# sanhue903/CUDA_Selection_Criteria

Measured on AMD Instinct MI355X. Metric: sketch pair-comparisons/sec (N genomes x m buckets), higher is better.
Workload: dtype u64; 1 GPU; cfg3: 10000 genomes, smh_a m=512, tau=0.8; mode smh_a; bands 64 x 8 rows; pair space sharded by query rows over 1 GPU(s), selected pairs all_gathered; n_genomes=10000, m=512, algo=sig, criterion=smh_a, selected_pairs=45000, stage1_survivors=45000, n_ranks_seen=1, stage2_grouping=label order

## Files before the change

cuda_selection_criteria_amd/csrc/abi_context.inc:

```

extern "C" {

const char* selhip_version(void) { return "selhip 0.1 (gfx950)"; }

int selhip_device_count(void) {
    int cnt = 0;
    if (hipGetDeviceCount(&cnt) != hipSuccess) return 0;
    return cnt;
}

const char* selhip_last_error(const selhip_ctx* ctx) {
    if (ctx) return ctx->err.c_str();
    return g_last_error.c_str();
}

int selhip_ctx_create(selhip_ctx** out, int device) {
    if (!out) return SELHIP_E_BADARG;
    *out = nullptr;
    int rc = check_device(nullptr);
    if (rc) return rc;
    int cnt = 0;
    (void)hipGetDeviceCount(&cnt);
    if (device < 0 || device >= cnt) { set_err(nullptr, "device %d out of range (0..%d)", device, cnt - 1); return SELHIP_E_BADARG; }
    HIPCHK(nullptr, hipSetDevice(device));
// ... 2 lines not shown
    if (std::strncmp(prop.gcnArchName, "gfx950", 6) != 0) {
        set_err(nullptr, "device %d is %s; this library is built for gfx950 only", device, prop.gcnArchName);
        return SELHIP_E_NODEVICE;
    }
    selhip_ctx* c = new selhip_ctx();
    c->device = device;
    c->dev_cus = prop.multiProcessorCount;
    *out = c;
    return SELHIP_OK;
}

void selhip_ctx_destroy(selhip_ctx* c) {
    if (!c) return;
    (void)hipSetDevice(c->device);
    (void)hipStreamSynchronize(c->stream);
    drain_timers(c);
    c->own_hll.release(); c->own_aux.release(); c->own_cards.release();
    c->ecard.release(); c->hi.release(); c->pc.buf.release(); c->seg_cnt.release(); c->surv.release();
    c->counts.release(); c->results.release(); c->self_pairs.release();
    c->aux_il.release(); c->cand.release(); c->sig.release(); c->fin.release(); c->own_aux_hll.release();
    c->hj_keys_in.release(); c->hj_keys_out.release(); c->hj_vals_in.release(); c->hj_vals_out.release(); c->hj_tmp.release();
    c->csr_cnt.release(); c->csr_start.release(); c->grouped.release(); c->scan_tmp.release();
    c->planes.release(); c->small_bar.release(); c->mat_row_pos.release(); c->mat_col_pos.release();
    c->hll_sparse.release(); c->hll_sparse_dev_t.release();
    release_queries(c);
    release_topk(c);
    c->gs.release();
    release_merge(c);
    if (c->h_pc) (void)hipHostFree(c->h_pc);
    if (c->st_stage1) {
        (void)hipStreamDestroy(c->st_stage1);
        (void)hipEventDestroy(c->ev_start); (void)hipEventDestroy(c->ev_end);
    }
    delete c;
}

int selhip_ctx_set_stream(selhip_ctx* c, void* hip_stream) {
    if (!c) return SELHIP_E_BADARG;
    if (c->stream != (hipStream_t)hip_stream && c->pc.buf.p) {
        (void)hipStreamSynchronize(c->stream);
        c->pc.dirty = true;
    }
    c->stream = (hipStream_t)hip_stream;
    return SELHIP_OK;
}

int selhip_ctx_set_fp_mode(selhip_ctx* c, int fp_mode) {
// ... 89 lines not shown
        return SELHIP_OK;
    }
    if (!std::strcmp(name, "query_join_tile")) {
        if (value != 16 && value != 32) { set_err(&c->err, "query_join_tile must be 16 or 32"); return SELHIP_E_BADARG; }
        c->query_join_tile = value;
        return SELHIP_OK;
    }
    if (!std::strcmp(name, "timed_kernel")) {
        if (value < 0 || value > 1) { set_err(&c->err, "timed_kernel must be 0 (stage-1 kernel) or 1 (stage 2a)"); return SELHIP_E_BADARG; }
        c->timed_kernel = value;
        return SELHIP_OK;
    }
    if (!std::strcmp(name, "hist_algo")) {
        if (value < -1 || value > 1) { set_err(&c->err, "hist_algo must be -1 (automatic), 0 (byte rows, LDS histogram) or 1 (bit planes)"); return SELHIP_E_BADARG; }
        c->hist_algo = value;
        if (value == 0) c->planes.khi = 0;
        return SELHIP_OK;
    }
    if (!std::strcmp(name, "hist_sparse")) {
        if (value < -1 || value > 1) { set_err(&c->err, "hist_sparse must be -1 (automatic), 0 (every value from the bit planes) or 1 (values >= the set's threshold from its sparse lists)"); return SELHIP_E_BADARG; }
        c->hist_sparse = value;
        return SELHIP_OK;
    }
    if (!std::strcmp(name, "dense_fused")) { c->dense_fused = value != 0; return SELHIP_OK; }
    if (!std::strcmp(name, "matrix_mirror")) { c->matrix_mirror = value != 0; return SELHIP_OK; }
    if (!std::strcmp(name, "matrix_smh_form")) {
        if (value != 1 && value != 3) { set_err(&c->err, "matrix_smh_form: 1 (every pair once, mirrored) or 3 (the whole square)"); return SELHIP_E_BADARG; }
        c->matrix_smh_form = (int)value; return SELHIP_OK;
    }
    if (!std::strcmp(name, "hist_dense_degree")) {
        if (value < -1 || value > (1 << 20)) { set_err(&c->err, "hist_dense_degree must be in [-1, 2^20] (-1 = never)"); return SELHIP_E_BADARG; }
        c->hist_dense_degree = value;
        return SELHIP_OK;
    }
    if (!std::strcmp(name, "hist_bs_blocks")) {
        if (value < 8 || value > 65536 || value % 8) { set_err(&c->err, "hist_bs_blocks must be a multiple of 8 in [8, 65536]"); return SELHIP_E_BADARG; }
        c->hist_bs_blocks = value;
        return SELHIP_OK;
    }
    if (!std::strcmp(name, "hist_blocks")) {
        if (value < 8 || value > 65536 || value % 8) { set_err(&c->err, "hist_blocks must be a multiple of 8 in [8, 65536]"); return SELHIP_E_BADARG; }
        c->hist_blocks = value;
        return SELHIP_OK;
    }
    if (!std::strcmp(name, "cluster_blocks")) {
        if (value < 0 || value > 65536) { set_err(&c->err, "cluster_blocks must be in [0, 65536] (0 = automatic)"); return SELHIP_E_BADARG; }
        g_cluster_blocks.store(value, std::memory_order_relaxed);
        return SELHIP_OK;
    }
    set_err(&c->err, "unknown parameter '%s'", name);
    return SELHIP_E_BADARG;
}

int selhip_ctx_get_param(const selhip_ctx* c, const char* name, int* value) {
    if (!c || !name || !value) return SELHIP_E_BADARG;
    if (!std::strcmp(name, "hll_khi"))          { *value = c->planes.khi; return SELHIP_OK; }
    if (!std::strcmp(name, "hist_bitplanes"))   { *value = use_bitslices(c) ? 1 : 0; return SELHIP_OK; }
    if (!std::strcmp(name, "hist_sparse_t"))    { *value = sparse_t_used(c); return SELHIP_OK; }
    if (!std::strcmp(name, "label_order"))      { *value = label_order(c) ? 1 : 0; return SELHIP_OK; }
    if (!std::strcmp(name, "join_tile_rows"))   { *value = join_tile_rows(c); return SELHIP_OK; }
    if (!std::strcmp(name, "join_form_used"))   { *value = c->join_form_used; return SELHIP_OK; }
    if (!std::strcmp(name, "chunks"))           { *value = c->n_chunks_last; return SELHIP_OK; }
    if (!std::strcmp(name, "dense_route_used")) { *value = c->dense_route_used; return SELHIP_OK; }
    if (!std::strcmp(name, "smhc_path_used"))   { *value = c->smhc_path_used; return SELHIP_OK; }
    if (!std::strcmp(name, "smhc_rule_used"))   { *value = c->smhc_rule_used; return SELHIP_OK; }
    if (!std::strcmp(name, "matrix_mirror"))    { *value = c->matrix_mirror; return SELHIP_OK; }
    if (!std::strcmp(name, "matrix_smh_form"))  { *value = c->matrix_smh_form; return SELHIP_OK; }
    if (!std::strcmp(name, "matrix_smh_path_used")) { *value = c->matrix_smh_path_used; return SELHIP_OK; }
    if (!std::strcmp(name, "clusters_last"))    { *value = c->clusters_last; return SELHIP_OK; }
    if (!std::strcmp(name, "cluster_blocks"))   { *value = g_cluster_blocks.load(std::memory_order_relaxed); return SELHIP_OK; }
    if (!std::strcmp(name, "greedy_clusters_last")) { *value = c->greedy_clusters_last; return SELHIP_OK; }
    if (!std::strcmp(name, "greedy_rounds_last"))   { *value = c->greedy_rounds_last; return SELHIP_OK; }
    if (!std::strcmp(name, "forest_rounds_last"))   { *value = c->forest_rounds_last; return SELHIP_OK; }
    if (!std::strcmp(name, "linkage_rounds_last"))  { *value = c->linkage_rounds_last; return SELHIP_OK; }
    if (!std::strcmp(name, "linkage_merges_last"))  { *value = c->linkage_merges_last; return SELHIP_OK; }
    if (!std::strcmp(name, "linkage_rowscans_last")) { *value = c->linkage_rowscans_last; return SELHIP_OK; }
    if (!std::strcmp(name, "linkage_rescans_last")) { *value = c->linkage_rescans_last; return SELHIP_OK; }
    if (!std::strcmp(name, "forest_edges_last"))    { *value = c->forest_edges_last; return SELHIP_OK; }
    if (!std::strcmp(name, "small_pass_used"))  { *value = c->small_used ? 1 : 0; return SELHIP_OK; }
    if (!std::strcmp(name, "pairs_route_used")) { *value = c->pairs_route_used; return SELHIP_OK; }
    if (!std::strcmp(name, "pairs_gpw"))        { *value = c->pairs_gpw_used; return SELHIP_OK; }
// ... 147 lines not shown
    return SELHIP_OK;
}

static int load_cards(selhip_ctx* c, const char* noun, const uint8_t* d_hll, int64_t n, const double* cards_src, bool cards_on_host,
                      DevBuf<double>& own, const double** d_cards, bool host_cards_checked = false) {
    if (!cards_src) {
        HIPCHK(&c->err, own.ensure((size_t)n));
        const int rc = compute_cards(c, d_hll, n, c->p, own.p);
        if (rc) return rc;
        *d_cards = own.p;
    } else if (cards_on_host) {
        if (!host_cards_checked) { const int rc = check_host_cards(c, noun, cards_src, n); if (rc) return rc; }
        HIPCHK(&c->err, own.ensure((size_t)n));
        HIPCHK(&c->err, hipMemcpyAsync(own.p, cards_src, (size_t)n * sizeof(double), hipMemcpyHostToDevice, c->stream));
        *d_cards = own.p;
    } else {
        *d_cards = cards_src;
    }
    HIPCHK(&c->err, hipStreamSynchronize(c->stream));
    return SELHIP_OK;
}

static int after_sketches(selhip_ctx* c, const double* cards_src, bool cards_on_host) {
    c->planes.khi = 0; c->hll_sparse_t = 0;
    if (c->n == 0) return SELHIP_OK;
    if (c->p == 14 && c->hist_algo != 0) {
        int rc = c->planes.build(&c->err, c->stream, c->d_hll, c->n);
        if (rc) return rc;
        HIPCHK(&c->err, c->hll_sparse.ensure((size_t)c->n * kBsSparseCap));
        HIPCHK(&c->err, c->hll_sparse_dev_t.ensure(1));
        rc = build_sparse_lists(&c->err, c->stream, c->planes.bs.p, c->n, c->hll_sparse.p, c->hll_sparse_dev_t.p, &c->hll_sparse_t);
        if (rc) return rc;
    }
    return load_cards(c, "cards", c->d_hll, c->n, cards_src, cards_on_host, c->own_cards, &c->d_cards, true);
}

static void set_database(selhip_ctx* c, int64_t n, int m, int p_hll) {
    c->n = n; c->m = m; c->p = p_hll; c->have_run = false; c->pending = false; c->cand_begin = 0; c->sig_key = 0; c->small_pass_failed = false;
    c->d_aux_hll = nullptr; c->p_aux = 0;
    drop_queries(c);
}

static int no_database(selhip_ctx* c, int rc) {
    c->n = 0; c->d_hll = nullptr; c->d_aux = nullptr; c->d_cards = nullptr; c->owns_sketches = false;
    c->planes.khi = 0; c->hll_sparse_t = 0;
    return rc;
}

static int upload_rows(selhip_ctx* c, const uint8_t* h_hll, const uint64_t* h_aux, const double* h_cards) {
    const size_t hb = (size_t)1 << c->p;
    if (c->n > 0) {
        HIPCHK(&c->err, c->own_hll.ensure((size_t)c->n * hb));
        HIPCHK(&c->err, c->own_aux.ensure((size_t)c->n * c->m));
        HIPCHK(&c->err, hipMemcpyAsync(c->own_hll.p, h_hll, (size_t)c->n * hb, hipMemcpyHostToDevice, c->stream));
        HIPCHK(&c->err, hipMemcpyAsync(c->own_aux.p, h_aux, (size_t)c->n * c->m * 8, hipMemcpyHostToDevice, c->stream));
    }
    c->d_hll = c->own_hll.p; c->d_aux = (const u64*)c->own_aux.p; c->owns_sketches = true;
    return after_sketches(c, h_cards, true);
}

int selhip_ctx_upload(selhip_ctx* c, const uint8_t* h_hll, const uint64_t* h_aux, const double* h_cards,
                      int64_t n, int m, int p_hll) {
    if (!c) return SELHIP_E_BADARG;
    HIPCHK(&c->err, hipSetDevice(c->device));
    int rc = validate_shape(c, n, m, p_hll);
    if (rc) return rc;
    if (n > 0 && (!h_hll || !h_aux)) { set_err(&c->err, "null sketch pointer"); return SELHIP_E_BADARG; }
    if (h_cards) { rc = check_host_cards(c, "cards", h_cards, n); if (rc) return rc; }
// ... 313 lines not shown
```

cuda_selection_criteria_amd/csrc/host_context.hpp:

```cpp
#pragma once

namespace {

thread_local std::string g_last_error = "";

void set_err(std::string* dst, const char* fmt, ...) {
    char buf[512];
    va_list ap;
    va_start(ap, fmt);
    vsnprintf(buf, sizeof buf, fmt, ap);
    va_end(ap);
    if (dst) *dst = buf;
    g_last_error = buf;
}

#define HIPCHK(ctx_err, expr)                                                                  \
    do {                                                                                       \
        hipError_t e__ = (expr);                                                               \
        if (e__ != hipSuccess) {                                                               \
            set_err(ctx_err, "%s failed: %s (%s:%d)", #expr, hipGetErrorString(e__), __FILE__, __LINE__); \
            return SELHIP_E_HIP;                                                               \
        }                                                                                      \
    } while (0)

// ... 153 lines not shown
    SigSet sig;
    DevBuf<u64> hj_keys_in, hj_keys_out;
    DevBuf<int> hj_vals_in, hj_vals_out;
    DevBuf<char> hj_tmp;
    DevBuf<int> csr_cnt, csr_start;
    DevBuf<selhip_int2_t> grouped;
    DevBuf<char> scan_tmp;
    size_t scan_tmp_stride = 0;
    PassCounters* h_pc = nullptr;
    hipStream_t st_stage1 = nullptr;
    hipEvent_t ev_start = nullptr, ev_end = nullptr;
    int n_chunks_last = 1;
    int pipeline = -1;
    int64_t cand_begin = 0;
    int il_block = 128, il_parts = 1, il_part = 0;
    int hist_pad = 0;
    int hist_run = 0, hist_blocks = kHistSpanBlocks;
    BitPlanes planes;
    DevBuf<u64> small_bar;
    DevBuf<uint32_t> hll_sparse;
    DevBuf<int> hll_sparse_dev_t;
    int hll_sparse_t = 0;
    int hist_sparse = -1;
    int hist_algo = -1;
    int hist_dense_degree = 32;
    int hist_bs_blocks = 2048;
    int group_label = -1;
    int verify_fb = 0;
    int join_wpb = 4;
    int join_db = 1;
    int join_tri = 0;
    int join_form = 2;
    int join_form_used = -1;
    int join_t = 0;
    int join_bits = 16;
    int join_q = 1;
    long long enum_pairs = kEnumPairs;
    int sig_tile_g = 16;
    int sig_cache = 0;
    long long sig_key = 0;
    int sig_tile = 1;
    int init_cap = 0;
    int join_qt = 0;
    bool group_stage2 = true;
    int small_pass = -1;
    bool small_used = false, small_pass_failed = false;
// ... 191 lines not shown
```

cuda_selection_criteria_amd/csrc/host_pairs.hpp:

```cpp
#pragma once

namespace {

constexpr long long kPairsSigShare = 2;

int pairs_route(const selhip_ctx* c, bool smh, int algo, int n_rows, int n_bands, int64_t n_pairs) {
    if (!smh) return 2;
    if (algo == SELHIP_ALGO_STREAM || !sig_supported(n_rows, n_bands)) return 0;
    if (algo == SELHIP_ALGO_SIG) return 1;
    const bool cached = c->sig_cache && c->sig_key == sig_cache_key(c, n_rows, n_bands);
    return cached || n_pairs >= c->n / kPairsSigShare ? 1 : 0;
}

hipError_t launch_pairs_filter(selhip_ctx* c, u64 off, u64 end, double tau, selhip_int2_t* out, u64 out_cap, u64* out_count, PassCounters* pc0) {
    const unsigned grid = grid_for(end - off, kPairsBlock, kPairsMaxGrid);
    if (off == 0) c->pairs_grid_used = (int)grid;
    hipLaunchKernelGGL(pairs_filter_kernel, dim3(grid), dim3(kPairsBlock), 0, c->stream,
                       c->list_pairs, off, end, (int)c->n, c->ecard.p, tau, c->mode == SELHIP_MODE_CB_SMH ? 1 : 0, out, out_cap, out_count, pc0);
    return hipGetLastError();
}

int enqueue_pairs_pass(selhip_ctx* c) {
    const int n = (int)c->n;
    const double tau = (double)c->tau_f;
    const int crit = c->criterion;
    const int use_cb = c->mode == SELHIP_MODE_CB_SMH ? 1 : 0;
    const u64 P = (u64)c->list_n;
    c->dominant_timer = c->timed_kernel == 1 ? T_HIST : T_STAGE1;
    if (c->timing) c->timed_passes += 1;
    TimerScope total(c, T_TOTAL);
    CounterSets::Claim pcs;
    HIPCHK(&c->err, c->pc.claim(c->stream, &pcs));
    c->pcb = pcs.cur;
    PassCounters* const pc0 = c->pcb;
    if (c->fail_after_flip) { c->fail_after_flip = 0; set_err(&c->err, "test hook: enqueue failed after the counter flip"); return SELHIP_E_HIP; }
    c->small_used = false;
    c->n_chunks_last = 1;
    if (c->pairs_route_used == 1) {
        HIPCHK(&c->err, launch_sig_build(c, c->n_rows, c->n_bands, tau, 0, 0, pcs.next));
    } else {
        TimerScope t(c, T_PREP);
        hipLaunchKernelGGL(cb_bounds_kernel, dim3((unsigned)((n + 255) / 256)), dim3(256), 0, c->stream,
                           c->d_cards, n, tau, use_cb, row_map(c, 0, 0), c->ecard.p, c->hi.p, pc0,
                           grouping_on(c) && !c->plan.emit ? c->csr_cnt.p : nullptr, grouping_on(c) && !c->plan.emit ? (int)c->csr_cnt.cap : 0, 0, pcs.next,
                           c->seg_cnt.p, (int)c->seg_cnt.cap);
        HIPCHK(&c->err, hipGetLastError());
    }
    const Chain ch = chain_slices(c, 0, 1, c->stream, 0, n, pc0, false);
    const StageIO& io = ch.io;
    const selhip_int2_t* final_list = io.surv;
    const u64* final_count = &io.pc->n_survivors;
    u64 final_cap = io.cap;
    if (c->plan.smh) {
        {
            TimerScope t(c, T_STAGE1);
            const unsigned grid = grid_for(P, kPairsBlock, kPairsMaxGrid);
            c->pairs_gpw_used = 0; c->pairs_grid_used = (int)grid;
            if (c->plan.count) {
                const PairsDirectShape sh = pairs_direct_shape(P);
// ... 61 lines not shown
```

cuda_selection_criteria_amd/csrc/host_pass.hpp:

```cpp
#pragma once

namespace {

template <int NCH, int LOG2R>
hipError_t launch_stream(selhip_ctx* c, const StageIO& io, const RowMap& rm) {
    constexpr int Q = kQueryVgprBudget / NCH;
    const int n = (int)c->n;
    const long long n_tiles_ll = rm.n_tiles(Q);
    if (n_tiles_ll > 0x7FFFFFFFll) return hipErrorInvalidValue;
    const int n_tiles = (int)n_tiles_ll;
    const int chunk_base = ((rm.row_begin + 1) / kChunk) * kChunk;
    const int n_chunks = (n - chunk_base + kChunk - 1) / kChunk;
    if (n_tiles <= 0 || n_chunks <= 0) return hipSuccess;
    const long long blocks = (long long)n_tiles * n_chunks;
    if (blocks > 0x7FFFFFFFll) return hipErrorInvalidValue;
    hipLaunchKernelGGL((smh_stream_kernel<NCH, LOG2R>), dim3((unsigned)blocks), dim3(kBlock), 0, io.st,
                       reinterpret_cast<const u64x2*>(c->aux_il.p), n, c->hi.p, c->pcb,
                       rm, n_tiles, chunk_base, io.surv, io.cap, io.pc);
    return hipGetLastError();
}

template <int NCH, int LOG2R>
hipError_t launch_stream_r(selhip_ctx* c, const StageIO& io, int l, const RowMap& rm) {
    if (l == LOG2R) return launch_stream<NCH, LOG2R>(c, io, rm);
// ... 377 lines not shown
template <int NB>
void launch_hist_bs_nb(int g1, unsigned blocks, hipStream_t st, const uint32_t* bs, const uint8_t* gmax, const uint32_t* lists, const selhip_int2_t* list,
                       const u64* count, u64 cap, uint32_t* counts, u64 off, u64 window, int run, u64 dense_pairs) {
#define SELHIP_BS_LAUNCH(G1) hipLaunchKernelGGL((hll_union_hist_bs_kernel<NB, G1>), dim3(blocks), dim3(kBlock), 0, st, bs, gmax, lists, list, count, cap, \
                                                counts, off, window, run, dense_pairs)
    switch (g1) {
        case 1: SELHIP_BS_LAUNCH(1); return;
        case 2: SELHIP_BS_LAUNCH(2); return;
        case 3: SELHIP_BS_LAUNCH(3); return;
    }
    if constexpr (NB > 4) {
        switch (g1) {
            case 4: SELHIP_BS_LAUNCH(4); return;
            case 5: SELHIP_BS_LAUNCH(5); return;
        }
    }
    if constexpr (NB > 5) {
        if (g1 == 6) { SELHIP_BS_LAUNCH(6); return; }
    }
    SELHIP_BS_LAUNCH(0);
#undef SELHIP_BS_LAUNCH
}
hipError_t launch_hist_bs(int khi, unsigned blocks, hipStream_t st, const uint32_t* bs, const uint8_t* gmax, const selhip_int2_t* list, const u64* count,
                          u64 cap, uint32_t* counts, u64 off, u64 window, int run, u64 dense_pairs, int sparse_t = 0, const uint32_t* lists = nullptr) {
    const int g1 = sparse_t > 0 && sparse_t < khi && lists ? sparse_t / 4 : 0;
    switch (bs_planes(khi)) {
        case 4:  launch_hist_bs_nb<4>(g1, blocks, st, bs, gmax, lists, list, count, cap, counts, off, window, run, dense_pairs); break;
        case 5:  launch_hist_bs_nb<5>(g1, blocks, st, bs, gmax, lists, list, count, cap, counts, off, window, run, dense_pairs); break;
        default: launch_hist_bs_nb<6>(g1, blocks, st, bs, gmax, lists, list, count, cap, counts, off, window, run, dense_pairs);
    }
    return hipGetLastError();
}

int build_sparse_lists(std::string* err, hipStream_t st, const uint32_t* d_bs, int64_t n, uint32_t* d_lists, int* d_t, int* t) {
    *t = 0;
    if (n <= 0) return SELHIP_OK;
    HIPCHK(err, hipMemsetAsync(d_t, 0, sizeof(int), st));
    hipLaunchKernelGGL(hll_sparse_t_kernel, dim3(grid_for((u64)n, kWavesPerBlock, 8192)), dim3(kBlock), 0, st, d_bs, (long long)n, d_t);
    HIPCHK(err, hipGetLastError());
    int need = 0;
    HIPCHK(err, hipMemcpyAsync(&need, d_t, sizeof(int), hipMemcpyDeviceToHost, st));
    HIPCHK(err, hipStreamSynchronize(st));
    if (need < 4 || need > kBsSparseMaxT) return SELHIP_OK;
    hipLaunchKernelGGL(hll_sparse_list_kernel, dim3(grid_for((u64)n, kWavesPerBlock, 8192)), dim3(kBlock), 0, st, d_bs, (long long)n, need, d_lists);
    HIPCHK(err, hipGetLastError());
    HIPCHK(err, hipStreamSynchronize(st));
    *t = need;
    return SELHIP_OK;
}

bool use_bitslices(const selhip_ctx* c) { return c->p == 14 && c->planes.khi > 0 && c->hist_algo != 0; }
constexpr size_t kSparseMaxPlaneBytes = (size_t)192 << 20;
int sparse_t_used(const selhip_ctx* c) {
    if (!use_bitslices(c) || !c->hist_sparse || c->hll_sparse_t >= c->planes.khi) return 0;
    if (c->hist_sparse < 0 && (size_t)c->n * kBsGenomeDwords * sizeof(uint32_t) > kSparseMaxPlaneBytes) return 0;
    if (c->hll_sparse_t > 20 && c->planes.khi <= 32) return 0;
    return c->hll_sparse_t;
}

int compute_cards(selhip_ctx* c, const uint8_t* d_hll, int64_t n, int p, double* d_out) {
    if (n <= 0) return SELHIP_OK;
    HIPCHK(&c->err, c->self_pairs.ensure((size_t)n));
    HIPCHK(&c->err, c->counts.ensure((size_t)n * 64));
    hipLaunchKernelGGL(iota_pairs_kernel, dim3((unsigned)((n + 255) / 256)), dim3(256), 0, c->stream, c->self_pairs.p, (int)n);
    HIPCHK(&c->err, hipGetLastError());
    hipLaunchKernelGGL(hll_union_hist_kernel, dim3(grid_for((u64)n, kWavesPerBlock, 4096)), dim3(kBlock), 0, c->stream,
                       d_hll, p, c->self_pairs.p, (const u64*)nullptr, (u64)n, (u64)n, c->counts.p);
    HIPCHK(&c->err, hipGetLastError());
    HIPCHK(&c->err, launch_select<0>(c->fp_mode == SELHIP_FP_FMA, c->stream, grid_for((u64)n, kWave, 8192), c->counts.p,
                                     nullptr, (u64)n, (u64)n, p, d_out, nullptr, nullptr, 0.0, nullptr, 0, nullptr,
                                     nullptr, nullptr));
    return SELHIP_OK;
}

long long pair_bound(long long n, long long rb, long long re) {
    long long cnt = 0;
    const long long rows = re - rb;
    cnt = rows * (n - 1) - (rb + re - 1) * rows / 2;
    return cnt < 0 ? 0 : cnt;
}

// ... 54 lines not shown
    selhip_int2_t* fin; u64 fin_cap;
    int* csr_cnt; int* csr_start; char* scan_tmp;
    selhip_int2_t* grouped;
    uint32_t* counts; u64 window;
};

size_t csr_stride(int n) { return 5 * (size_t)n + 2; }

constexpr double kLabelOrderPairs = 4e8;
constexpr size_t kLabelOrderBytes = (size_t)192 << 20;
bool label_order(const selhip_ctx* c) {
    if (!grouping_on(c)) return false;
    if (c->group_label >= 0) return c->group_label == 1;
    if (use_bitslices(c)) return true;
    return (size_t)c->n * 16384 > kLabelOrderBytes && (double)pair_bound(c->n, c->row_begin, c->row_end) / std::max(1, c->il_parts) >= kLabelOrderPairs;
}

int enqueue_hist_select(selhip_ctx* c, const Chain& ch, const selhip_int2_t* final_list, const u64* final_count, u64 final_cap,
                        bool grouped, double tau, PassCounters* pc0) {
    hipStream_t st = ch.io.st;
    for (u64 off = 0; off < final_cap; off += ch.window) {
        {
            TimerScope t(c, T_HIST, st);
            if (use_bitslices(c))
                HIPCHK(&c->err, launch_hist_bs(c->planes.khi, (unsigned)c->hist_bs_blocks, st, c->planes.bs.p, c->planes.gmax.p, final_list, final_count, final_cap, ch.counts, off, ch.window,
                                               c->hist_run > 0 ? c->hist_run : (grouped ? 4 : 1),
                                               grouped && c->hist_dense_degree >= 0
                                                   ? (u64)c->hist_dense_degree * (u64)std::max<long long>(1, ((long long)ch.re - ch.rb) / std::max(1, c->il_parts)) : ~0ull,
                                               sparse_t_used(c), c->hll_sparse.p));
            else if (c->p == 14)
                hipLaunchKernelGGL(hll_union_hist_runs_kernel, dim3(c->hist_blocks), dim3(kWave), (size_t)c->hist_pad, st,
                                   c->d_hll, final_list, final_count, final_cap, ch.counts, off, ch.window,
                                   c->hist_run > 0 ? c->hist_run : (grouped && label_order(c) ? 4 : 1));
            else
                hipLaunchKernelGGL(hll_union_hist_kernel, dim3(2048), dim3(kBlock), 0, st,
                                   c->d_hll, c->p, final_list, final_count, (u64)0, final_cap, ch.counts, off, ch.window);
            HIPCHK(&c->err, hipGetLastError());
        }
        TimerScope t(c, T_SELECT, st);
        HIPCHK(&c->err, launch_select<1>(c->fp_mode == SELHIP_FP_FMA, st, 4096, ch.counts, final_count, 0,
                                         final_cap, c->p, nullptr, final_list, c->ecard.p, tau,
                                         c->results.p, (u64)c->results.cap, pc0, nullptr, nullptr, off, ch.window, c->measure));
    }
    return SELHIP_OK;
}

int enqueue_tail(selhip_ctx* c, const Chain& ch, const selhip_int2_t* final_list, const u64* final_count, u64 final_cap,
                 bool counted, double tau, PassCounters* pc0) {
    const int n = (int)c->n;
    hipStream_t st = ch.io.st;
    const bool grouped = grouping_on(c);
    if (grouped) {
// ... 176 lines not shown
    ch.counts = c->counts.p + (size_t)k * ch.window * 64;
    if (count_in_verify) { ch.io.row_cnt = ch.csr_cnt; if (label_order(c)) ch.io.row_lab = ch.csr_cnt + 2 * (size_t)n; }
    return ch;
}

int enqueue_pass(selhip_ctx* c) {
    const int n = (int)c->n;
    const int rb = (int)(c->rd.on ? c->rd.begin : c->row_begin), re = (int)(c->rd.on ? c->rd.end : c->row_end);
    const double tau = (double)c->tau_f;
    const int crit = c->criterion;
    const PassPlan& plan = c->plan;
    c->dominant_timer = c->timed_kernel == 1 ? T_HIST : crit == SELHIP_CRIT_NONE ? T_DENSE : (plan.use_sig ? T_JOIN : T_STAGE1);
    if (c->timing && !(c->rd.on && c->rd.begin != c->row_begin)) c->timed_passes += 1;
    TimerScope total(c, T_TOTAL);
    const bool smh_crit = plan.smh, use_hash = plan.use_hash, use_sig = plan.use_sig;
    if (plan.bad) { set_err(&c->err, plan.bad, c->n_rows, c->n_bands); return SELHIP_E_BADARG; }
    CounterSets::Claim pcs;
    HIPCHK(&c->err, c->pc.claim(c->stream, &pcs));
    c->pcb = pcs.cur;
    PassCounters* const pc_next = pcs.next;
    PassCounters* pc0 = c->pcb;
    if (c->fail_after_flip) { c->fail_after_flip = 0; set_err(&c->err, "test hook: enqueue failed after the counter flip"); return SELHIP_E_HIP; }
    c->small_used = small_pass_ok(c);
    if (c->small_used) {
        c->n_chunks_last = 1;
        const int rc = enqueue_small_pass(c, pc_next, tau);
        if (rc) return rc;
        HIPCHK(&c->err, hipMemcpyAsync(c->h_pc, c->pcb, sizeof(PassCounters) * (kMaxChunks + 1), hipMemcpyDeviceToHost, c->stream));
        c->pc.dirty = false;
        return SELHIP_OK;
    }
    if (use_sig) {
        HIPCHK(&c->err, launch_sig_build(c, c->n_rows, c->n_bands, tau, rb, re, pc_next));
    } else {
        TimerScope t(c, T_PREP);
        hipLaunchKernelGGL(cb_bounds_kernel, dim3((unsigned)((n + 255) / 256)), dim3(256), 0, c->stream,
                           c->d_cards, n, tau, c->mode == SELHIP_MODE_CB_SMH ? 1 : 0, row_map(c, rb, re), c->ecard.p, c->hi.p, pc0,
                           grouping_on(c) && !plan.emit ? c->csr_cnt.p : nullptr, grouping_on(c) && !plan.emit ? (int)c->csr_cnt.cap : 0, (int)c->cand_begin, pc_next,
                           c->seg_cnt.p, (int)c->seg_cnt.cap);
        HIPCHK(&c->err, hipGetLastError());
        if (plan.il_stream) {
            const int nch = c->m / 128;
            const long long total = (long long)c->n * nch * kWave;
            hipLaunchKernelGGL(stream_interleave_kernel, dim3((unsigned)((total + kBlock - 1) / kBlock)), dim3(kBlock), 0, c->stream,
                               reinterpret_cast<const u64x2*>(c->d_aux), reinterpret_cast<u64x2*>(c->aux_il.p), total, nch);
            HIPCHK(&c->err, hipGetLastError());
// ... 146 lines not shown
```

cuda_selection_criteria_amd/csrc/kernel_hllbs.cuh:

```cuda
#pragma once

namespace {

constexpr int kBsPlanes = 6;
constexpr int kBsPlaneDwords = 512;
constexpr int kBsGenomeDwords = kBsPlanes * kBsPlaneDwords;

__global__ __launch_bounds__(kBlock)
void hll_bitslice_kernel(const uint8_t* __restrict__ hll, long long n, uint32_t* __restrict__ bs, uint8_t* __restrict__ gmax,
                         int* __restrict__ max_val) {
    const int lane = threadIdx.x & (kWave - 1);
    uint32_t mx_all = 0;
    for (long long g = (long long)blockIdx.x * kWavesPerBlock + threadIdx.x / kWave; g < n; g += (long long)gridDim.x * kWavesPerBlock) {
        const uint32_t* row = reinterpret_cast<const uint32_t*>(hll + g * 16384);
        uint32_t* dst = bs + g * kBsGenomeDwords;
        uint32_t mx = 0;
#pragma unroll 1
        for (int o = 0; o < 8; ++o) {
            uint32_t d[8];
#pragma unroll
            for (int jj = 0; jj < 8; ++jj) d[jj] = row[(o * 8 + jj) * kWave + lane] & 0x3F3F3F3Fu;
            uint32_t out[kBsPlanes];
#pragma unroll
            for (int b = 0; b < kBsPlanes; ++b) out[b] = 0;
#pragma unroll
            for (int jj = 0; jj < 8; ++jj) {
                const uint32_t w = d[jj];
                mx = max(max(mx, w & 0xFFu), max((w >> 8) & 0xFFu, max((w >> 16) & 0xFFu, w >> 24)));
#pragma unroll
// ... 30 lines not shown
        int cnt[6] = {0, 0, 0, 0, 0, 0};
#pragma unroll 1
        for (int o = 0; o < kBsPlaneDwords / kWave; ++o) {
            uint32_t p[kBsPlanes];
#pragma unroll
            for (int b = 0; b < kBsPlanes; ++b) p[b] = src[b * kBsPlaneDwords + o * kWave + lane];
#pragma unroll
            for (int k = 1; k <= 6; ++k) cnt[k - 1] += __popc(bs_ge4k(p, k));
        }
        int t = kBsSparseMaxT + 4;
#pragma unroll
        for (int k = 6; k >= 1; --k) {
            int s = cnt[k - 1];
#pragma unroll
            for (int d = 32; d > 0; d >>= 1) s += __shfl_xor(s, d, kWave);
            if (s <= kBsSparseCap) t = 4 * k;
        }
        t_all = max(t_all, t);
    }
    if (lane == 0 && t_all) atomicMax(t_need, t_all);
}

__global__ __launch_bounds__(kBlock)
void hll_sparse_list_kernel(const uint32_t* __restrict__ bs, long long n, int t, uint32_t* __restrict__ lists) {
    const int lane = threadIdx.x & (kWave - 1);
    for (long long g = (long long)blockIdx.x * kWavesPerBlock + threadIdx.x / kWave; g < n; g += (long long)gridDim.x * kWavesPerBlock) {
        const uint32_t* src = bs + g * kBsGenomeDwords;
        uint32_t* dst = lists + g * kBsSparseCap;
        int base = 0;
#pragma unroll 1
        for (int o = 0; o < kBsPlaneDwords / kWave; ++o) {
            const int d = o * kWave + lane;
            uint32_t p[kBsPlanes];
#pragma unroll
            for (int b = 0; b < kBsPlanes; ++b) p[b] = src[b * kBsPlaneDwords + d];
            uint32_t h = bs_ge4k(p, t >> 2);
            const int cnt = __popc(h);
            int incl = cnt;
#pragma unroll
            for (int s = 1; s < kWave; s <<= 1) {
                const int v = __shfl_up(incl, s, kWave);
                if (lane >= s) incl += v;
            }
            int off = base + incl - cnt;
            while (h) {
                const int j = __builtin_ctz(h);
                h &= h - 1;
                uint32_t v = 0;
#pragma unroll
                for (int b = 0; b < kBsPlanes; ++b) v |= ((p[b] >> j) & 1u) << b;
                if (off < kBsSparseCap) dst[off] = ((uint32_t)(d * 32 + j) << 8) | v;
                ++off;
            }
            base += __shfl(incl, kWave - 1, kWave);
        }
        for (int i = lane; i < kBsSparseCap; i += kWave)
            if (i >= base) dst[i] = kBsSparseNone;
    }
}

template <int NB>
__device__ __forceinline__ void bs_load(const uint32_t* __restrict__ bs, int g, int lane, uint32_t (&r)[NB][8]) {
    const uint4* p = reinterpret_cast<const uint4*>(bs + (size_t)g * kBsGenomeDwords);
#pragma unroll
    for (int b = 0; b < NB; ++b) {
        const uint4 lo = p[b * (kBsPlaneDwords / 4) + lane], hi = p[b * (kBsPlaneDwords / 4) + kWave + lane];
        r[b][0] = lo.x; r[b][1] = lo.y; r[b][2] = lo.z; r[b][3] = lo.w;
        r[b][4] = hi.x; r[b][5] = hi.y; r[b][6] = hi.z; r[b][7] = hi.w;
    }
}

template <int TBL>
__device__ __forceinline__ uint32_t bs_op3(uint32_t a, uint32_t b, uint32_t c) { return __builtin_amdgcn_bitop3_b32(a, b, c, TBL); }
__device__ __forceinline__ void bs_count(uint32_t& acc, uint32_t mask) {
    asm("v_bcnt_u32_b32 %0, %1, %0" : "+v"(acc) : "v"(mask));
}

template <int NB, int G>
__device__ __forceinline__ uint32_t bs_group_node(const uint32_t (&M)[NB], const uint32_t (&pre)[4]) {
    constexpr int s1 = (G & 2) ? 0xCC : 0x33, s0 = (G & 1) ? 0xAA : 0x55;
    if constexpr (NB == 4)      return bs_op3<((G & 2) ? 0xF0 : 0x0F) & ((G & 1) ? 0xCC : 0x33)>(M[3], M[2], M[2]);
    else if constexpr (NB == 5) return bs_op3<((G & 4) ? 0xF0 : 0x0F) & s1 & s0>(M[4], M[3], M[2]);
    else                        return bs_op3<0xF0 & s1 & s0>(pre[G >> 2], M[3], M[2]);
}

template <int NB, int G0, int G, int GEND>
// ... 150 lines not shown
    }
    const uint32_t hA = sp->bins[my_bin];
    sp->bins[my_bin] = 0u;
    __builtin_amdgcn_fence(__ATOMIC_RELEASE, "wavefront");
    __builtin_amdgcn_wave_barrier();
    __builtin_amdgcn_fence(__ATOMIC_ACQUIRE, "wavefront");
    return hA;
}

__device__ __forceinline__ void bs_sparse_entry(BsSparseLds* sp, uint32_t e) {
    if (e == kBsSparseNone) return;
    const uint32_t r = e >> 8, v = e & 63, w = sp->bits[r >> 5], below = w & ((1u << (r & 31)) - 1u);
    if ((w >> (r & 31)) & 1u) {
        const uint32_t av = sp->val[sp->first[r >> 5] + __popc(below)];
        if (v > av) {
            atomicAdd(&sp->bins[v], 1u);
            atomicSub(&sp->bins[av], 1u);
        }
    } else {
        atomicAdd(&sp->bins[v], 1u);
    }
}

template <int NB, int G1>
__global__ __launch_bounds__(kBlock, NB <= 5 ? 4 : 2)
void hll_union_hist_bs_kernel(const uint32_t* __restrict__ bs, const uint8_t* __restrict__ gmax, const uint32_t* __restrict__ lists,
                              const selhip_int2_t* __restrict__ pairs, const u64* __restrict__ n_pairs_dev, u64 cap, uint32_t* __restrict__ counts,
                              u64 chunk_off, u64 chunk_len, int run_len, u64 dense_pairs) {
    const int lane = threadIdx.x & (kWave - 1);
    const int wave = threadIdx.x / kWave;
    u64 n_pairs = *n_pairs_dev;
    if (n_pairs > cap) n_pairs = cap;
    n_pairs = n_pairs > chunk_off ? min(n_pairs - chunk_off, chunk_len) : 0;
    pairs += chunk_off;
    u64 blocks_active = gridDim.x;
    {
        const u64 resident = 1024ull * (NB <= 5 ? 4 : 2);
        if (n_pairs <= 8 * resident) {
            const u64 waves = min(resident, max(n_pairs, (u64)64));
            blocks_active = min((u64)gridDim.x, ((waves + 8 * kWavesPerBlock - 1) / (8 * kWavesPerBlock)) * 8);
        }
    }
    if (blockIdx.x >= blocks_active) return;
    const u64 stride = (blocks_active >> 3) * kWavesPerBlock;
    const int my_bin = ((lane & 2) ? 32 : 0) + 2 * bs_pidx(lane) + (lane & 1);
    const bool dense = n_pairs >= dense_pairs;
    const uint32_t xcd = blockIdx.x & 7u;
// ... 4 lines not shown
    const u64 n_tasks = (n_pairs + run_len - 1) / run_len;
    const u64 tasks_per_xcd = dense ? n_tasks : (n_tasks + 7) >> 3;
    const u64 t_begin = dense ? 0 : (u64)xcd * tasks_per_xcd, t_end = min(t_begin + tasks_per_xcd, n_tasks);
    int cur_x = -1;
    uint32_t xa[NB][8];
    BsSparseLds* sp = nullptr;
    uint32_t hA = 0;
    if constexpr (G1 > 0) {
        __shared__ BsSparseLds sp_block[kWavesPerBlock];
        sp = &sp_block[wave];
        sp->bins[my_bin] = 0u;
    }
    for (u64 task = t_begin + (u64)(blockIdx.x >> 3) * kWavesPerBlock + wave; task < t_end; task += stride) {
        const u64 j0 = task * run_len;
        const int cnt = (int)min((u64)run_len, n_pairs - j0);
        selhip_int2_t pr{0, 0};
        if (lane < cnt) pr = pairs[j0 + lane];
        u64 mine = __ballot(lane < cnt && (!dense || (((uint32_t)pr.y * 0x9E3779B1u) >> 29) == xcd));
        while (mine) {
            const int src = (int)__builtin_ctzll(mine);
            mine &= mine - 1;
            const int px = __builtin_amdgcn_readlane(pr.x, src), py = __builtin_amdgcn_readlane(pr.y, src);
            uint32_t yb[NB][8];
            bs_load<NB>(bs, py, lane, yb);
            if constexpr (G1 == 0) {
                if (px != cur_x) { bs_load<NB>(bs, px, lane, xa); cur_x = px; }
                const int kp = max((int)gmax[px], (int)gmax[py]) + 1;
                const uint32_t tot = bs_pair_hist<NB>(xa, yb, kp, lane);
                counts[(j0 + src) * 64 + my_bin] = (lane & 1) ? (tot >> 16) : (tot & 0xFFFFu);
            } else {
                const uint32_t eb0 = lists[(size_t)py * kBsSparseCap + lane], eb1 = lists[(size_t)py * kBsSparseCap + kWave + lane];
                if (px != cur_x) { bs_load<NB>(bs, px, lane, xa); hA = bs_sparse_row(sp, lists, px, lane, my_bin); cur_x = px; }
                uint32_t P[16];
#pragma unroll
                for (int v = 0; v < 16; ++v) P[v] = 0u;
                bs_decode<NB, 0, G1, 16>(xa, yb, P);
                const uint32_t tot = bs_reduce16<2 * G1>(P, lane);
                bs_sparse_entry(sp, eb0);
                bs_sparse_entry(sp, eb1);
                __builtin_amdgcn_fence(__ATOMIC_RELEASE, "wavefront");
                __builtin_amdgcn_wave_barrier();
                __builtin_amdgcn_fence(__ATOMIC_ACQUIRE, "wavefront");
                const uint32_t s = sp->bins[my_bin];
                sp->bins[my_bin] = 0u;
                const uint32_t dense_cnt = (lane & 2) ? 0u : ((lane & 1) ? (tot >> 16) : (tot & 0xFFFFu));
                counts[(j0 + src) * 64 + my_bin] = dense_cnt + hA + s;
            }
        }
    }
}


}
```

Measured before the change: 279.4 billion pairs/s.

## Add clamped four-plane HLL image to shrink sparse histogram kernel loads

```diff
diff --git a/cuda_selection_criteria_amd/csrc/abi_context.inc b/cuda_selection_criteria_amd/csrc/abi_context.inc
--- a/cuda_selection_criteria_amd/csrc/abi_context.inc
+++ b/cuda_selection_criteria_amd/csrc/abi_context.inc
@@ -48,7 +48,7 @@
     c->hj_keys_in.release(); c->hj_keys_out.release(); c->hj_vals_in.release(); c->hj_vals_out.release(); c->hj_tmp.release();
     c->csr_cnt.release(); c->csr_start.release(); c->grouped.release(); c->scan_tmp.release();
     c->planes.release(); c->small_bar.release(); c->mat_row_pos.release(); c->mat_col_pos.release();
-    c->hll_sparse.release(); c->hll_sparse_dev_t.release();
+    c->hll_sparse.release(); c->hll_sparse_dev_t.release(); c->hll_image.release();
     release_queries(c);
     release_topk(c);
     c->gs.release();
@@ -184,6 +184,11 @@
         c->hist_sparse = value;
         return SELHIP_OK;
     }
+    if (!std::strcmp(name, "hist_image")) {
+        if (value < -1 || value > 1) { set_err(&c->err, "hist_image must be -1 (automatic), 0 (the six-plane rows) or 1 (the clamped image where the set holds one)"); return SELHIP_E_BADARG; }
+        c->hist_image = value;
+        return SELHIP_OK;
+    }
     if (!std::strcmp(name, "dense_fused")) { c->dense_fused = value != 0; return SELHIP_OK; }
     if (!std::strcmp(name, "matrix_mirror")) { c->matrix_mirror = value != 0; return SELHIP_OK; }
     if (!std::strcmp(name, "matrix_smh_form")) {
@@ -219,6 +224,7 @@
     if (!std::strcmp(name, "hll_khi"))          { *value = c->planes.khi; return SELHIP_OK; }
     if (!std::strcmp(name, "hist_bitplanes"))   { *value = use_bitslices(c) ? 1 : 0; return SELHIP_OK; }
     if (!std::strcmp(name, "hist_sparse_t"))    { *value = sparse_t_used(c); return SELHIP_OK; }
+    if (!std::strcmp(name, "hist_image"))       { *value = c->hist_image_used; return SELHIP_OK; }
     if (!std::strcmp(name, "label_order"))      { *value = label_order(c) ? 1 : 0; return SELHIP_OK; }
     if (!std::strcmp(name, "join_tile_rows"))   { *value = join_tile_rows(c); return SELHIP_OK; }
     if (!std::strcmp(name, "join_form_used"))   { *value = c->join_form_used; return SELHIP_OK; }
@@ -412,14 +418,14 @@
 }
 
 static int after_sketches(selhip_ctx* c, const double* cards_src, bool cards_on_host) {
-    c->planes.khi = 0; c->hll_sparse_t = 0;
+    c->planes.khi = 0; c->hll_sparse_t = 0; c->hll_image_ok = false;
     if (c->n == 0) return SELHIP_OK;
     if (c->p == 14 && c->hist_algo != 0) {
         int rc = c->planes.build(&c->err, c->stream, c->d_hll, c->n);
         if (rc) return rc;
         HIPCHK(&c->err, c->hll_sparse.ensure((size_t)c->n * kBsSparseCap));
         HIPCHK(&c->err, c->hll_sparse_dev_t.ensure(1));
-        rc = build_sparse_lists(&c->err, c->stream, c->planes.bs.p, c->n, c->hll_sparse.p, c->hll_sparse_dev_t.p, &c->hll_sparse_t);
+        rc = build_sparse_lists(&c->err, c->stream, c->planes.bs.p, c->n, c->hll_sparse.p, c->hll_sparse_dev_t.p, &c->hll_sparse_t, &c->hll_image, &c->hll_image_ok);
         if (rc) return rc;
     }
     return load_cards(c, "cards", c->d_hll, c->n, cards_src, cards_on_host, c->own_cards, &c->d_cards, true);
@@ -433,7 +439,7 @@
 
 static int no_database(selhip_ctx* c, int rc) {
     c->n = 0; c->d_hll = nullptr; c->d_aux = nullptr; c->d_cards = nullptr; c->owns_sketches = false;
-    c->planes.khi = 0; c->hll_sparse_t = 0;
+    c->planes.khi = 0; c->hll_sparse_t = 0; c->hll_image_ok = false;
     return rc;
 }
 
diff --git a/cuda_selection_criteria_amd/csrc/host_context.hpp b/cuda_selection_criteria_amd/csrc/host_context.hpp
--- a/cuda_selection_criteria_amd/csrc/host_context.hpp
+++ b/cuda_selection_criteria_amd/csrc/host_context.hpp
@@ -199,6 +199,10 @@
     DevBuf<int> hll_sparse_dev_t;
     int hll_sparse_t = 0;
     int hist_sparse = -1;
+    DevBuf<uint32_t> hll_image;
+    bool hll_image_ok = false;
+    int hist_image = -1;
+    int hist_image_used = 0;
     int hist_algo = -1;
     int hist_dense_degree = 32;
     int hist_bs_blocks = 2048;
diff --git a/cuda_selection_criteria_amd/csrc/host_pairs.hpp b/cuda_selection_criteria_amd/csrc/host_pairs.hpp
--- a/cuda_selection_criteria_amd/csrc/host_pairs.hpp
+++ b/cuda_selection_criteria_amd/csrc/host_pairs.hpp
@@ -35,6 +35,7 @@
     PassCounters* const pc0 = c->pcb;
     if (c->fail_after_flip) { c->fail_after_flip = 0; set_err(&c->err, "test hook: enqueue failed after the counter flip"); return SELHIP_E_HIP; }
     c->small_used = false;
+    c->hist_image_used = 0;
     c->n_chunks_last = 1;
     if (c->pairs_route_used == 1) {
         HIPCHK(&c->err, launch_sig_build(c, c->n_rows, c->n_bands, tau, 0, 0, pcs.next));
diff --git a/cuda_selection_criteria_amd/csrc/host_pass.hpp b/cuda_selection_criteria_amd/csrc/host_pass.hpp
--- a/cuda_selection_criteria_amd/csrc/host_pass.hpp
+++ b/cuda_selection_criteria_amd/csrc/host_pass.hpp
@@ -423,8 +423,20 @@
 #undef SELHIP_BS_LAUNCH
 }
 hipError_t launch_hist_bs(int khi, unsigned blocks, hipStream_t st, const uint32_t* bs, const uint8_t* gmax, const selhip_int2_t* list, const u64* count,
-                          u64 cap, uint32_t* counts, u64 off, u64 window, int run, u64 dense_pairs, int sparse_t = 0, const uint32_t* lists = nullptr) {
+                          u64 cap, uint32_t* counts, u64 off, u64 window, int run, u64 dense_pairs, int sparse_t = 0, const uint32_t* lists = nullptr,
+                          const uint32_t* image = nullptr) {
     const int g1 = sparse_t > 0 && sparse_t < khi && lists ? sparse_t / 4 : 0;
+    if (image && g1 >= 1 && 4 * g1 <= kBsImageMaxT) {
+#define SELHIP_BS_IMAGE(G1) hipLaunchKernelGGL((hll_union_hist_bs_kernel<kBsImagePlanes, G1, kBsImageDwords>), dim3(blocks), dim3(kBlock), 0, st, image, gmax, lists, \
+                                               list, count, cap, counts, off, window, run, dense_pairs)
+        switch (g1) {
+            case 1:  SELHIP_BS_IMAGE(1); break;
+            case 2:  SELHIP_BS_IMAGE(2); break;
+            default: SELHIP_BS_IMAGE(3);
+        }
+#undef SELHIP_BS_IMAGE
+        return hipGetLastError();
+    }
     switch (bs_planes(khi)) {
         case 4:  launch_hist_bs_nb<4>(g1, blocks, st, bs, gmax, lists, list, count, cap, counts, off, window, run, dense_pairs); break;
         case 5:  launch_hist_bs_nb<5>(g1, blocks, st, bs, gmax, lists, list, count, cap, counts, off, window, run, dense_pairs); break;
@@ -433,8 +445,10 @@
     return hipGetLastError();
 }
 
-int build_sparse_lists(std::string* err, hipStream_t st, const uint32_t* d_bs, int64_t n, uint32_t* d_lists, int* d_t, int* t) {
+int build_sparse_lists(std::string* err, hipStream_t st, const uint32_t* d_bs, int64_t n, uint32_t* d_lists, int* d_t, int* t, DevBuf<uint32_t>* image,
+                       bool* image_ok) {
     *t = 0;
+    *image_ok = false;
     if (n <= 0) return SELHIP_OK;
     HIPCHK(err, hipMemsetAsync(d_t, 0, sizeof(int), st));
     hipLaunchKernelGGL(hll_sparse_t_kernel, dim3(grid_for((u64)n, kWavesPerBlock, 8192)), dim3(kBlock), 0, st, d_bs, (long long)n, d_t);
@@ -443,21 +457,27 @@
     HIPCHK(err, hipMemcpyAsync(&need, d_t, sizeof(int), hipMemcpyDeviceToHost, st));
     HIPCHK(err, hipStreamSynchronize(st));
     if (need < 4 || need > kBsSparseMaxT) return SELHIP_OK;
-    hipLaunchKernelGGL(hll_sparse_list_kernel, dim3(grid_for((u64)n, kWavesPerBlock, 8192)), dim3(kBlock), 0, st, d_bs, (long long)n, need, d_lists);
+    const bool with_image = need <= kBsImageMaxT;
+    if (with_image) HIPCHK(err, image->ensure((size_t)n * kBsImageDwords));
+    hipLaunchKernelGGL(hll_sparse_list_kernel, dim3(grid_for((u64)n, kWavesPerBlock, 8192)), dim3(kBlock), 0, st, d_bs, (long long)n, need, d_lists,
+                       with_image ? image->p : nullptr);
     HIPCHK(err, hipGetLastError());
     HIPCHK(err, hipStreamSynchronize(st));
     *t = need;
+    *image_ok = with_image;
     return SELHIP_OK;
 }
 
 bool use_bitslices(const selhip_ctx* c) { return c->p == 14 && c->planes.khi > 0 && c->hist_algo != 0; }
+bool image_ready(const selhip_ctx* c) { return c->hist_image != 0 && c->hll_image_ok && c->hll_sparse_t >= 4 && c->hll_sparse_t <= kBsImageMaxT; }
 constexpr size_t kSparseMaxPlaneBytes = (size_t)192 << 20;
 int sparse_t_used(const selhip_ctx* c) {
     if (!use_bitslices(c) || !c->hist_sparse || c->hll_sparse_t >= c->planes.khi) return 0;
-    if (c->hist_sparse < 0 && (size_t)c->n * kBsGenomeDwords * sizeof(uint32_t) > kSparseMaxPlaneBytes) return 0;
+    if (c->hist_sparse < 0 && !image_ready(c) && (size_t)c->n * kBsGenomeDwords * sizeof(uint32_t) > kSparseMaxPlaneBytes) return 0;
     if (c->hll_sparse_t > 20 && c->planes.khi <= 32) return 0;
     return c->hll_sparse_t;
 }
+bool image_used(const selhip_ctx* c) { return image_ready(c) && sparse_t_used(c) == c->hll_sparse_t; }
 
 int compute_cards(selhip_ctx* c, const uint8_t* d_hll, int64_t n, int p, double* d_out) {
     if (n <= 0) return SELHIP_OK;
@@ -558,12 +578,13 @@
     for (u64 off = 0; off < final_cap; off += ch.window) {
         {
             TimerScope t(c, T_HIST, st);
+            if (use_bitslices(c)) c->hist_image_used = image_used(c) ? 1 : 0;
             if (use_bitslices(c))
                 HIPCHK(&c->err, launch_hist_bs(c->planes.khi, (unsigned)c->hist_bs_blocks, st, c->planes.bs.p, c->planes.gmax.p, final_list, final_count, final_cap, ch.counts, off, ch.window,
                                                c->hist_run > 0 ? c->hist_run : (grouped ? 4 : 1),
                                                grouped && c->hist_dense_degree >= 0
                                                    ? (u64)c->hist_dense_degree * (u64)std::max<long long>(1, ((long long)ch.re - ch.rb) / std::max(1, c->il_parts)) : ~0ull,
-                                               sparse_t_used(c), c->hll_sparse.p));
+                                               sparse_t_used(c), c->hll_sparse.p, image_used(c) ? c->hll_image.p : nullptr));
             else if (c->p == 14)
                 hipLaunchKernelGGL(hll_union_hist_runs_kernel, dim3(c->hist_blocks), dim3(kWave), (size_t)c->hist_pad, st,
                                    c->d_hll, final_list, final_count, final_cap, ch.counts, off, ch.window,
@@ -786,6 +807,7 @@
     PassCounters* pc0 = c->pcb;
     if (c->fail_after_flip) { c->fail_after_flip = 0; set_err(&c->err, "test hook: enqueue failed after the counter flip"); return SELHIP_E_HIP; }
     c->small_used = small_pass_ok(c);
+    c->hist_image_used = 0;
     if (c->small_used) {
         c->n_chunks_last = 1;
         const int rc = enqueue_small_pass(c, pc_next, tau);
diff --git a/cuda_selection_criteria_amd/csrc/kernel_hllbs.cuh b/cuda_selection_criteria_amd/csrc/kernel_hllbs.cuh
--- a/cuda_selection_criteria_amd/csrc/kernel_hllbs.cuh
+++ b/cuda_selection_criteria_amd/csrc/kernel_hllbs.cuh
@@ -5,6 +5,9 @@
 constexpr int kBsPlanes = 6;
 constexpr int kBsPlaneDwords = 512;
 constexpr int kBsGenomeDwords = kBsPlanes * kBsPlaneDwords;
+constexpr int kBsImagePlanes = 4;
+constexpr int kBsImageDwords = kBsImagePlanes * kBsPlaneDwords;
+constexpr int kBsImageMaxT = 12;
 
 __global__ __launch_bounds__(kBlock)
 void hll_bitslice_kernel(const uint8_t* __restrict__ hll, long long n, uint32_t* __restrict__ bs, uint8_t* __restrict__ gmax,
@@ -81,7 +84,7 @@
 }
 
 __global__ __launch_bounds__(kBlock)
-void hll_sparse_list_kernel(const uint32_t* __restrict__ bs, long long n, int t, uint32_t* __restrict__ lists) {
+void hll_sparse_list_kernel(const uint32_t* __restrict__ bs, long long n, int t, uint32_t* __restrict__ lists, uint32_t* __restrict__ image) {
     const int lane = threadIdx.x & (kWave - 1);
     for (long long g = (long long)blockIdx.x * kWavesPerBlock + threadIdx.x / kWave; g < n; g += (long long)gridDim.x * kWavesPerBlock) {
         const uint32_t* src = bs + g * kBsGenomeDwords;
@@ -93,6 +96,11 @@
             uint32_t p[kBsPlanes];
 #pragma unroll
             for (int b = 0; b < kBsPlanes; ++b) p[b] = src[b * kBsPlaneDwords + d];
+            if (image) {
+                const uint32_t top = p[4] | p[5];
+#pragma unroll
+                for (int b = 0; b < kBsImagePlanes; ++b) image[g * kBsImageDwords + b * kBsPlaneDwords + d] = p[b] | top;
+            }
             uint32_t h = bs_ge4k(p, t >> 2);
             const int cnt = __popc(h);
             int incl = cnt;
@@ -118,9 +126,10 @@
     }
 }
 
-template <int NB>
+template <int NB, int PITCH = kBsGenomeDwords>
 __device__ __forceinline__ void bs_load(const uint32_t* __restrict__ bs, int g, int lane, uint32_t (&r)[NB][8]) {
-    const uint4* p = reinterpret_cast<const uint4*>(bs + (size_t)g * kBsGenomeDwords);
+    static_assert(NB * kBsPlaneDwords <= PITCH, "a row holds the planes read");
+    const uint4* p = reinterpret_cast<const uint4*>(bs + (size_t)g * PITCH);
 #pragma unroll
     for (int b = 0; b < NB; ++b) {
         const uint4 lo = p[b * (kBsPlaneDwords / 4) + lane], hi = p[b * (kBsPlaneDwords / 4) + kWave + lane];
@@ -317,7 +326,7 @@
     }
 }
 
-template <int NB, int G1>
+template <int NB, int G1, int PITCH = kBsGenomeDwords>
 __global__ __launch_bounds__(kBlock, NB <= 5 ? 4 : 2)
 void hll_union_hist_bs_kernel(const uint32_t* __restrict__ bs, const uint8_t* __restrict__ gmax, const uint32_t* __restrict__ lists,
                               const selhip_int2_t* __restrict__ pairs, const u64* __restrict__ n_pairs_dev, u64 cap, uint32_t* __restrict__ counts,
@@ -368,15 +377,15 @@
             mine &= mine - 1;
             const int px = __builtin_amdgcn_readlane(pr.x, src), py = __builtin_amdgcn_readlane(pr.y, src);
             uint32_t yb[NB][8];
-            bs_load<NB>(bs, py, lane, yb);
+            bs_load<NB, PITCH>(bs, py, lane, yb);
             if constexpr (G1 == 0) {
-                if (px != cur_x) { bs_load<NB>(bs, px, lane, xa); cur_x = px; }
+                if (px != cur_x) { bs_load<NB, PITCH>(bs, px, lane, xa); cur_x = px; }
                 const int kp = max((int)gmax[px], (int)gmax[py]) + 1;
                 const uint32_t tot = bs_pair_hist<NB>(xa, yb, kp, lane);
                 counts[(j0 + src) * 64 + my_bin] = (lane & 1) ? (tot >> 16) : (tot & 0xFFFFu);
             } else {
                 const uint32_t eb0 = lists[(size_t)py * kBsSparseCap + lane], eb1 = lists[(size_t)py * kBsSparseCap + kWave + lane];
-                if (px != cur_x) { bs_load<NB>(bs, px, lane, xa); hA = bs_sparse_row(sp, lists, px, lane, my_bin); cur_x = px; }
+                if (px != cur_x) { bs_load<NB, PITCH>(bs, px, lane, xa); hA = bs_sparse_row(sp, lists, px, lane, my_bin); cur_x = px; }
                 uint32_t P[16];
 #pragma unroll
                 for (int v = 0; v < 16; ++v) P[v] = 0u;
```

Result: faster. 284.2 billion pairs/s, median of 6 (+1.7%).
